# sozoluffy/TensorNetworks

Measured on AMD Instinct MI355X. Metric: ksd_gradient_steps_per_sec, higher is better.
Workload: dtype f64; 1 GPU; n16_L6_dense; n_qubits=16, layers=6, ansatz=hardware_efficient, params=288, gram=dense, bayesian_network=synthetic n=16 seed=0 (SURVEY 8d), optimizer=adam lr=0.005 cosine clip=10, parallelism=paramshift + gram row shard x1

## Files before the change

### tensornetworks_amd/csrc/plan.cpp

```cpp
#include "plan.hpp"

#include <algorithm>
#include <array>
#include <cstring>
#include <utility>

namespace bornvi {

int num_params(int ansatz, int n, int layers) {
  if (ansatz == 0 || ansatz == 1) return layers * 3 * n;
  if (ansatz == 2) return layers * 2 * n;
  return -1;
}

bool build_gate_list(int ansatz, int n, int layers, std::vector<Gate>& g) {
  g.clear();
  int p = 0;
  auto rot = [&](int kind, int w) { g.push_back({kind, w, -1, p++}); };
  if (ansatz == 0) {
    for (int i = 0; i < n; ++i) g.push_back({G_H, i, -1, -1});
    for (int l = 0; l < layers; ++l) {
      for (int i = 0; i < n; ++i) { rot(G_RX, i); rot(G_RY, i); rot(G_RZ, i); }
      if (n > 1) {
        for (int i = 0; i + 1 < n; ++i) g.push_back({G_CNOT, i, i + 1, -1});
// ... 180 lines not shown
}

std::vector<int> order_for_banks(std::vector<int> pos) {
  std::sort(pos.begin(), pos.end());
  std::vector<int> out;
  std::vector<char> used(pos.size(), 0);
  bool res_used[4] = {false, false, false, false};
  auto take = [&](auto pred) -> bool {
    for (size_t i = 0; i < pos.size(); ++i)
      if (!used[i] && pred(pos[i])) { used[i] = 1; out.push_back(pos[i]); res_used[pos[i] & 3] = true; return true; }
    return false;
  };
  for (int s = 0; s < 3 && out.size() < pos.size(); ++s)
    if (!take([&](int p) { return (p & 3) != 3 && !res_used[p & 3]; }))
      take([&](int) { return true; });
  if (out.size() < pos.size())
    if (!take([&](int p) { return (p & 3) == 3; })) take([&](int) { return true; });
  if (out.size() < pos.size() && out.size() >= 2) {
    int r0 = out[0] & 3, r1 = out[1] & 3;
    if (!take([&](int p) { return (p & 3) == r0 || (p & 3) == r1; })) take([&](int) { return true; });
  }
  for (size_t i = 0; i < pos.size(); ++i)
    if (!used[i]) out.push_back(pos[i]);
  return out;
}

void split_pass_ops(const std::vector<Op>& ops, const std::vector<int>& pass_ops, int n, bool is_init,
                    std::vector<int>& lead, std::vector<int>& core, std::vector<int>& trail) {
  lead.clear(); core.clear(); trail.clear();
  std::vector<char> touched(n, 0);
  std::vector<int> mid;
  for (int idx : pass_ops) {
    const Op& o = ops[idx];
    if (!is_init && o.kind == K_CX && !touched[o.a] && !touched[o.b]) { lead.push_back(idx); continue; }
    touched[o.a] = 1; if (o.b >= 0) touched[o.b] = 1;
    mid.push_back(idx);
  }
  std::fill(touched.begin(), touched.end(), 0);
  std::vector<int> trail_rev, core_rev;
  for (size_t q = mid.size(); q-- > 0;) {
    const Op& o = ops[mid[q]];
    if (o.kind == K_CX && !touched[o.a] && !touched[o.b]) { trail_rev.push_back(mid[q]); continue; }
    touched[o.a] = 1; if (o.b >= 0) touched[o.b] = 1;
    core_rev.push_back(mid[q]);
  }
  core.assign(core_rev.rbegin(), core_rev.rend());
  trail.assign(trail_rev.rbegin(), trail_rev.rend());
}

int count_stages(const std::vector<Op>& ops, const std::vector<int>& core, int n, int r, bool defer_cx3, bool read_map) {
  std::vector<int> pool = core, rest;
  int cnt = 0;
  while (!pool.empty()) {
    StageSel sel;
    stage_select(ops, pool, n, r, sel, rest, defer_cx3, read_map);
    if (sel.count() == 0) return 1 << 20;
    ++cnt;
    pool = rest;
  }
  return cnt;
}
bool pick_defer_policy(const std::vector<Op>& ops, const std::vector<int>& core, int n, int r, bool read_map) {
  return read_map && count_stages(ops, core, n, r, true, true) < count_stages(ops, core, n, r, false, true);
}

void first_last_stage_targets(const std::vector<Op>& ops, const std::vector<int>& pass_ops, int n, int r, bool is_init,
                              std::vector<int>& first_t, std::vector<int>& last_t, bool read_map) {
  std::vector<int> lead, core, trail, rest;
  split_pass_ops(ops, pass_ops, n, is_init, lead, core, trail);
  first_t.clear(); last_t.clear();
  std::vector<int> pool = core;
  bool first = true;
  const bool defer = pick_defer_policy(ops, core, n, r, read_map);
  while (!pool.empty()) {
    StageSel sel;
    stage_select(ops, pool, n, r, sel, rest, defer, read_map);
    if (sel.count() == 0) break;
    if (first) { first_t = sel.targets; first = false; }
    last_t = sel.targets;
    pool = rest;
  }
}

struct PassInfo {
  std::vector<int> ops;
  std::vector<int> targets;
  std::vector<int> local;
  std::vector<int> global;
  std::vector<int> lds_wire;
  std::vector<int> in_low;
  std::vector<int> out_low;
};

}

namespace {
struct BuildSpec {
  int n = 0;
  std::vector<Op> ops;
  std::vector<Fused> fused;
  int n_params = 0, n_gates = 0;
  bool in_state = false;
  bool out_state = false;
  std::vector<std::pair<int, int>> out_perm;
};
bool build_plan(const BuildSpec& spec, const PlanOptions& opt, Plan& plan, std::string& msg);
}

namespace {
bool make_plan_impl(int ansatz, int n, int layers, const PlanOptions& opt, Plan& plan, std::string& msg, std::vector<TailOp>* tail);
}

bool make_plan(int ansatz, int n, int layers, const PlanOptions& opt, Plan& plan, std::string& msg) {
  return make_plan_impl(ansatz, n, layers, opt, plan, msg, nullptr);
}

bool make_state_plan(int ansatz, int n, int layers, const PlanOptions& opt, Plan& plan, std::vector<TailOp>& tail, std::string& msg) {
  tail.clear();
  return make_plan_impl(ansatz, n, layers, opt, plan, msg, &tail);
}

namespace {
bool make_plan_impl(int ansatz, int n, int layers, const PlanOptions& opt, Plan& plan, std::string& msg, std::vector<TailOp>* tail) {
  if (n < 1 || n > MAX_PLAN_QUBITS) { msg = "num qubits must be in [1, " + std::to_string(MAX_PLAN_QUBITS) + "]"; return false; }
  if (layers < 0) { msg = "layers must be >= 0"; return false; }
  std::vector<Gate> gates;
  if (!build_gate_list(ansatz, n, layers, gates)) { msg = "unknown ansatz id"; return false; }
  BuildSpec spec;
  spec.n = n;
  fuse_gates(gates, n, spec.ops, spec.fused);
  {
    size_t last_u = spec.ops.size();
    while (last_u > 0 && spec.ops[last_u - 1].kind != K_U1) --last_u;
    for (size_t q = last_u; q < spec.ops.size(); ++q) {
      if (tail) tail->push_back({spec.ops[q].kind == K_CZ ? 1 : 0, spec.ops[q].a, spec.ops[q].b});
      else if (spec.ops[q].kind == K_CX) spec.out_perm.push_back({spec.ops[q].a, spec.ops[q].b});
    }
    spec.ops.resize(last_u);
  }
  spec.out_state = tail != nullptr;
  spec.n_params = num_params(ansatz, n, layers);
  spec.n_gates = (int)gates.size();
  if (opt.kmulti == 0 && n > opt.kmax && opt.kmax >= 13) {
    PlanOptions o11 = opt, o13 = opt;
    o11.kmulti = 11;
    o13.kmulti = 13;
    if (opt.r == 3) return build_plan(spec, o13, plan, msg);
    Plan p13;
    std::string m13;
    if (build_plan(spec, o13, p13, m13)) {
      FastTables ft;
      if ((build_fast_tables(p13, FAST_TABLE_MAX_BYTES, ft) && p13.fast_lds_bytes(ft.max_tab_rows) <= MAX_LDS_BYTES) ||
          n - o11.kmulti > 16) {
        plan = std::move(p13);
        return true;
      }
    }
    return build_plan(spec, o11, plan, msg);
  }
  return build_plan(spec, opt, plan, msg);
}
}

bool make_kron_plan(int n, const PlanOptions& opt, Plan& plan, std::string& msg) {
  if (n < 1 || n > MAX_PLAN_QUBITS) { msg = "num bits must be in [1, " + std::to_string(MAX_PLAN_QUBITS) + "]"; return false; }
  BuildSpec spec;
  spec.n = n;
  Fused f; f.fill(0xffffffffu); f[0] = 0; f[1] = 0;
  spec.fused.push_back(f);
  for (int w = n - 1; w >= 0; --w) spec.ops.push_back({K_U1, w, -1, 0});
  spec.in_state = spec.out_state = true;
  spec.n_gates = n;
  if (opt.kmulti == 0 && n - 12 > 16 && opt.kmax >= 13) {
    PlanOptions o13 = opt;
    o13.kmulti = 13;
    return build_plan(spec, o13, plan, msg);
  }
  return build_plan(spec, opt, plan, msg);
}

namespace {
bool build_plan(const BuildSpec& spec, const PlanOptions& opt, Plan& plan, std::string& msg) {
  const int n = spec.n;
  const std::vector<Op>& ops = spec.ops;
  const std::vector<Fused>& fused = spec.fused;
  const int kmulti = opt.kmulti > 0 ? opt.kmulti : (n <= 16 ? 11 : 12);
  const int k = (n <= opt.kmax) ? n : std::min(opt.kmax, kmulti);
  const int r = std::min(opt.r, k);
  if (r > 4) { msg = "at most 4 register wires"; return false; }
  int threads = 64;
  while (threads < (1 << (k - r))) threads <<= 1;
  if (threads > opt.max_threads) { msg = "tile needs more threads than allowed"; return false; }
  if (fused.size() > 65535) { msg = "too many fused gates"; return false; }

  std::vector<PassInfo> passes;
  {
    std::vector<int> pool(ops.size());
    for (size_t i = 0; i < ops.size(); ++i) pool[i] = (int)i;
    std::vector<int> sel, rest, tg;
    while (!pool.empty()) {
      choose_pass(ops, pool, n, k, sel, rest, tg);
      if (sel.empty()) { msg = "planner made no progress"; return false; }
      PassInfo pi; pi.ops = sel; pi.targets = tg;
      passes.push_back(pi);
      pool = rest;
    }
    if (passes.empty()) passes.push_back(PassInfo{});
  }
  const int lo_can = std::min(opt.lo, k);
  std::vector<int> canon_low;
  for (int p = 0; p < lo_can; ++p) canon_low.push_back(n - 1 - p);
  std::vector<int> canon_low_out = canon_low;
  {
    auto count_with = [&](int lo) {
      std::vector<char> in(n, 0);
      int cnt = 0;
      for (int w : passes.back().targets) { in[w] = 1; ++cnt; }
      for (int p = 0; p < lo; ++p) if (!in[n - 1 - p]) { in[n - 1 - p] = 1; ++cnt; }
      return cnt;
    };
    int lo_fit = -1;
    for (int lo = lo_can; lo >= std::min(3, lo_can); --lo)
      if (count_with(lo) <= k) { lo_fit = lo; break; }
    if (lo_fit < 0) passes.push_back(PassInfo{});
    else canon_low_out.resize(lo_fit);
  }
  if (spec.in_state) {
    std::vector<char> in(n, 0);
    int cnt = 0;
    for (int w : passes.front().targets) { in[w] = 1; ++cnt; }
    for (int w : canon_low) if (!in[w]) { in[w] = 1; ++cnt; }
    if (cnt > k) passes.insert(passes.begin(), PassInfo{});
  }
  const int np = (int)passes.size();
  for (int i = 0; i < np; ++i) {
    PassInfo& P = passes[i];
    std::vector<char> in(n, 0);
    auto add = [&](int w) { if (!in[w] && (int)P.local.size() < k) { in[w] = 1; P.local.push_back(w); } };
    for (int w : P.targets) add(w);
    if (i == np - 1) for (int w : canon_low_out) add(w);
    if (i == 0 && spec.in_state) for (int w : canon_low) add(w);
    if (i + 1 < np) for (int w : passes[i + 1].targets) add(w);
    if (i > 0) for (int w : passes[i - 1].local) add(w);
    for (int w = n - 1; w >= 0; --w) add(w);
    for (int w = 0; w < n; ++w) if (!in[w]) P.global.push_back(w);
  }
  if (spec.in_state) passes[0].in_low = canon_low;
  for (int i = 0; i < np; ++i) {
    PassInfo& P = passes[i];
    std::vector<char> placed(n, 0);
    for (int w : P.in_low) { P.lds_wire.push_back(w); placed[w] = 1; }
    std::vector<int> others;
    for (int w : P.local) if (!placed[w]) others.push_back(w);
    std::sort(others.begin(), others.end());
    for (int w : others) P.lds_wire.push_back(w);
    if (i == np - 1) { P.out_low = canon_low_out; break; }
    std::vector<char> nxt(n, 0);
    for (int w : passes[i + 1].local) nxt[w] = 1;
    std::vector<int> ldspos(n, -1);
    for (int j = 0; j < k; ++j) ldspos[P.lds_wire[j]] = j;
    std::vector<int> pos;
    for (int w : P.local) if (nxt[w]) pos.push_back(ldspos[w]);
    {
      std::vector<int> f_cur, l_cur, f_nxt, l_nxt;
      first_last_stage_targets(ops, P.ops, n, r, i == 0 && !spec.in_state, f_cur, l_cur, opt.use_read_map());
      first_last_stage_targets(ops, passes[i + 1].ops, n, r, false, f_nxt, l_nxt, opt.use_read_map());
      std::vector<char> busy(n, 0);
      for (int w : l_cur) busy[w] = 1;
      for (int w : f_nxt) busy[w] = 1;
      std::vector<int> quiet;
      for (int q : pos) if (!busy[P.lds_wire[q]]) quiet.push_back(q);
      if ((int)quiet.size() >= std::min(4, std::min(opt.lo, k))) pos = quiet;
    }
    pos = order_for_banks(pos);
    const int lo = std::min((int)pos.size(), std::min(opt.lo, k));
    for (int j = 0; j < lo; ++j) P.out_low.push_back(P.lds_wire[pos[j]]);
    passes[i + 1].in_low = P.out_low;
  }
  std::vector<std::vector<int>> layout(np, std::vector<int>(n, -1));
  for (int i = 0; i < np; ++i) {
    if (i == np - 1) { for (int w = 0; w < n; ++w) layout[i][w] = n - 1 - w; continue; }
    int p = 0;
    for (int w : passes[i].out_low) layout[i][w] = p++;
    if (opt.contig_out) {
      std::vector<char> nxt(n, 0);
      for (int w : passes[i + 1].local) nxt[w] = 1;
      for (int w : passes[i].local) if (layout[i][w] < 0 && nxt[w]) layout[i][w] = p++;
      for (int w : passes[i].local) if (layout[i][w] < 0) layout[i][w] = p++;
    }
    for (int w = 0; w < n; ++w) if (layout[i][w] < 0) layout[i][w] = p++;
  }
// ... 469 lines not shown
        const uint32_t* RWL = W.data() + rw_base + (size_t)(nst - 1) * per_stage;
        bool ok = (n + sh) <= 32;
        uint32_t basis[4] = {0, 0, 0, 0};
        for (int b = 0; b < r; ++b) basis[b] = phys_v(inv[W[hbase + FH_WORDS + (size_t)(nst - 1) * FS_WORDS + FS_WB + b] >> 4]) << sh;
        const uint32_t lanes_o = 1u << std::min<uint32_t>(P[PW_LO_OUT], 6u);
        const uint32_t runmask = (lanes_o << sh) - 1u;
        if (P[PW_LO_OUT] < 4u && !(pflags & PASS_FINAL)) ok = false;
        if ((pflags & PASS_FINAL) && P[PW_LO_OUT] < 3u) ok = false;
        for (uint32_t g = 0; g < ngl && ok; ++g) {
          uint32_t gslot = 0, gphys = 0;
          for (int m = 0; m < n - k; ++m) if (g >> m & 1) { gslot ^= thalf(PW_OUT_GMASK, m); gphys ^= P[PW_OUT_GCOL + m]; }
          for (uint32_t t = 0; t < (1u << kt2); ++t) {
            const uint32_t wslot = RWL[((size_t)g << kt2) + t] >> 16;
            W[tab + ((size_t)g << kt2) + t] = (phys_v(inv[wslot ^ gslot]) ^ gphys) << sh;
          }
          for (uint32_t t0 = 0; t0 < (1u << kt2) && ok; t0 += lanes_o) {
            uint32_t runs[2] = {0, 0};
            int nruns = 0;
            uint64_t seen = 0;
            for (uint32_t l = 0; l < lanes_o; ++l) {
              const uint32_t o = W[tab + ((size_t)g << kt2) + t0 + l];
              const uint32_t rb = o & ~runmask;
              int f = -1;
              for (int q = 0; q < nruns; ++q) if (runs[q] == rb) f = q;
              if (f < 0) { if (nruns == 2) { ok = false; break; } runs[nruns++] = rb; }
              seen |= 1ull << ((o >> sh) & (lanes_o - 1u));
            }
            if (nruns > ((pflags & PASS_FINAL) ? 2 : 1)) ok = false;
            if (seen != (lanes_o == 64 ? ~0ull : ((1ull << lanes_o) - 1ull))) ok = false;
          }
        }
        if (ok) {
          W[hbase + FH_OUT_TAB] = tab;
          for (int b = 0; b < r; ++b) W[hbase + FH_OUT_BASIS + b] = basis[b];
        } else {
          W.resize(tab);
        }
      }
    }
  }
  return true;
}


namespace {
inline uint32_t par32(uint32_t v) { return (uint32_t)__builtin_popcount(v) & 1u; }

struct StageEval {
  const uint32_t* S = nullptr;
  const uint32_t* tab = nullptr;
  const uint32_t* Qpre = nullptr;
  const uint32_t* Qpost = nullptr;
  uint32_t sri[3] = {0, 0, 0}, rpos[3] = {0, 0, 0};
  int k = 0, n = 0;
  uint32_t rw(uint32_t g, uint32_t t, uint32_t* e_out = nullptr, uint32_t* e2_out = nullptr) const {
    const uint32_t pb = tab[t] & 0xffffu, base = tab[t] >> 16;
    const uint32_t e = base | (g << k);
    uint32_t lflip = 0, sflip = 0, e2 = e;
    for (int b = 0; b < 3; ++b) {
      if (par32(e & S[8 + b])) lflip ^= sri[b];
      if (par32(e & S[12 + b])) { sflip ^= sri[b]; e2 |= 1u << rpos[b]; }
    }
    for (int p2 = 0; p2 < k; ++p2)
      if (S[48 + p2] && par32(e & S[48 + p2])) lflip ^= lds_swizzle(1u << p2);
    if (e_out) *e_out = e;
    if (e2_out) *e2_out = e2;
    return (pb ^ lflip) | ((pb ^ sflip) << 16);
  }
  uint32_t sign_bits(const uint32_t* Q, uint32_t e) const {
    uint32_t acc = 0;
    for (int q = 0; q < n; ++q) acc ^= ((e >> q) & 1u) & par32(e & Q[q]);
    uint32_t m = 0;
    for (int j = 0; j < 16; ++j) m |= (((Q[48] >> j) ^ acc ^ par32(e & Q[32 + j])) & 1u) << j;
    return m;
  }
  uint32_t sg(uint32_t g, uint32_t t) const {
    uint32_t e, e2;
    (void)rw(g, t, &e, &e2);
    return (Qpre ? sign_bits(Qpre, e) : 0u) | ((Qpost ? sign_bits(Qpost, e2) : 0u) << 16);
  }
};
}

bool build_compact_tables(const Plan& plan, CompactTables& out, std::string& msg) {
  out = CompactTables();
  const int n = plan.n, k = plan.k, r = plan.r;
  if (r != 3) { msg = "compact tables: the plan must have 3 register wires"; return false; }
  if (k < 6 || plan.threads != std::max(64, 1 << (k - 3)) || n - k > 16 || n > 27) { msg = "compact tables: tile below 2^6 or state too large"; return false; }
  const int kt = k - 3, gbits = n - k;
  const uint32_t T = 1u << kt, NW = std::max(T / 64u, 1u), ngl = 1u << gbits, ksize = 1u << k;
  std::vector<uint32_t>& W = out.words;
  auto fail = [&](const std::string& m) { msg = "compact tables: " + m; out = CompactTables(); return false; };
  for (int i = 0; i < plan.n_passes; ++i) {
    const uint32_t* P = plan.words.data() + plan.pass_off[i];
    const uint32_t nst = P[PW_NSTAGES];
    if (nst > (uint32_t)MAX_STAGES) return fail("too many stages");
    auto tbyte = [&](int table, int j) { return (P[table + (j >> 2)] >> (8 * (j & 3))) & 0xffu; };
    auto thalf = [&](int table, int j) { return (P[table + (j >> 1)] >> (16 * (j & 1))) & 0xffffu; };
    const uint32_t pflags = P[PW_FLAGS];
    const int out_shift = (pflags & PASS_FINAL) ? 3 : 4;
    std::vector<StageEval> SE(nst);
    uint32_t sign_pre = 0, sign_post = 0;
    {
      const uint32_t* S = P + PW_STAGES;
      for (uint32_t s = 0; s < nst; ++s) {
        const uint32_t hdr = S[0], sflags = (hdr >> 8) & 0xffu, rho = S[1];
        if ((hdr & 0xffu) != 3u) return fail("a stage with r != 3");
        StageEval& E = SE[s];
        E.S = S; E.k = k; E.n = n;
        for (int b = 0; b < 3; ++b) { E.rpos[b] = (rho >> (8 * b)) & 0xffu; E.sri[b] = lds_swizzle(1u << E.rpos[b]); }
        E.Qpre = (sflags & STAGE_SIGN_PRE) ? S + STAGE_HDR_WORDS : nullptr;
        E.Qpost = (sflags & STAGE_SIGN_POST) ? S + STAGE_HDR_WORDS + (E.Qpre ? SIGNQ_WORDS : 0) : nullptr;
        E.tab = S + STAGE_HDR_WORDS + (E.Qpre ? SIGNQ_WORDS : 0) + (E.Qpost ? SIGNQ_WORDS : 0);
        if (E.Qpre) sign_pre |= 1u << s;
        if (E.Qpost) sign_post |= 1u << s;
        S += hdr >> 16;
      }
    }
    const uint32_t sign_any = sign_pre | sign_post;
    const uint32_t nsign = (uint32_t)__builtin_popcount(sign_any);
    const uint32_t nrows = nst + nsign + CR_EXTRA;
    const uint32_t hb = (uint32_t)W.size();
    out.pass_off.push_back(hb);
    W.resize(hb + CH_WORDS + (size_t)nst * CS_WORDS, 0);
    W[hb + CH_NSTAGES] = nst; W[hb + CH_NROWS] = nrows; W[hb + CH_NSIGN] = nsign;
    W[hb + CH_SIGN_PRE] = sign_pre; W[hb + CH_SIGN_POST] = sign_post; W[hb + CH_NWAVES] = NW;
    for (uint32_t s = 0; s < nst; ++s) {
      const uint32_t* S = SE[s].S;
      const uint32_t sflags = (S[0] >> 8) & 0xffu;
      const uint32_t fi[4] = {S[6] & 0xffffu, S[6] >> 16, S[7] & 0xffffu, S[7] >> 16};
      uint32_t ngt = 0;
      while (ngt < 3 && fi[ngt] != 0xffffu) ++ngt;
      for (uint32_t b = ngt; b < 4; ++b) if (fi[b] != 0xffffu) return fail("gates not on register bits 0 .. ng-1");
      uint32_t* CS = W.data() + hb + CH_WORDS + (size_t)s * CS_WORDS;
      CS[CS_KIND] = ngt | ((sflags & STAGE_SIGN_PRE) ? 8u : 0u) | ((sflags & STAGE_SIGN_POST) ? 16u : 0u);
      CS[CS_CROSS] = (sflags & STAGE_CROSS_READ) ? 1u : 0u;
      for (int b = 0; b < 3; ++b) {
        CS[CS_RB + b] = S[16 + (1 << b)] << 4; CS[CS_WB + b] = S[32 + (1 << b)] << 4;
        CS[CS_MAT + b] = (fi[b] != 0xffffu ? fi[b] : 0u) * 64u;
      }
      for (int j = 0; j < 8; ++j) {
        uint32_t lr = 0, lw = 0;
        for (int b = 0; b < 3; ++b) if (j >> b & 1) { lr ^= S[16 + (1 << b)]; lw ^= S[32 + (1 << b)]; }
        if (lr != S[16 + j] || lw != S[32 + j]) return fail("slot offsets not linear in the slot number");
      }
    }
    W[hb + CH_MAT_OFF] = (uint32_t)W.size() - hb;
    {
      uint32_t nmat = 0;
      for (uint32_t s = 0; s < nst; ++s) {
        const uint32_t* S = SE[s].S;
        const uint32_t fi[3] = {S[6] & 0xffffu, S[6] >> 16, S[7] & 0xffffu};
        for (int b = 0; b < 3; ++b) if (fi[b] != 0xffffu) { W.push_back(fi[b] * 64u); ++nmat; }
      }
      W[hb + CH_NMAT] = nmat;
    }
    for (int m = 0; m < 3; ++m) {
      W[hb + CH_IN_STEP_N + m] = 16u << tbyte(PW_IN_PHYS, kt + m);
      W[hb + CH_FILL_STEP + m] = thalf(PW_IN_MASK, kt + m);
      W[hb + CH_DRAIN_STEP + m] = thalf(PW_OUT_MASK, kt + m);
      W[hb + CH_OUT_STEP_N + m] = P[PW_OUT_COL + kt + m] << out_shift;
    }
    std::vector<uint32_t> inv_in, inv_out;
    bool ok_in = false, ok_out = false;
    uint32_t in_basis[3] = {0, 0, 0}, out_basis[3] = {0, 0, 0};
    auto in_slot_lin = [&](uint32_t u) { uint32_t o = 0; for (int j = 0; j < k; ++j) if (u >> j & 1) o ^= thalf(PW_IN_MASK, j); return o; };
    auto in_phys_u = [&](uint32_t u) { uint32_t o = 0; for (int j = 0; j < k; ++j) if (u >> j & 1) o |= 1u << tbyte(PW_IN_PHYS, j); return o; };
    auto out_slot_lin = [&](uint32_t v) { uint32_t o = 0; for (int j = 0; j < k; ++j) if (v >> j & 1) o ^= thalf(PW_OUT_MASK, j); return o; };
    auto out_phys_v = [&](uint32_t v) { uint32_t o = 0; for (int j = 0; j < k; ++j) if (v >> j & 1) o ^= P[PW_OUT_COL + j]; return o; };
    auto g_in = [&](uint32_t g, uint32_t& gslot, uint32_t& gphys) {
      gslot = gphys = 0;
      for (int m = 0; m < gbits; ++m) if (g >> m & 1) { gslot ^= thalf(PW_IN_GMASK, m); gphys |= 1u << tbyte(PW_IN_GPHYS, m); }
    };
    auto g_out = [&](uint32_t g, uint32_t& gslot, uint32_t& gphys) {
      gslot = gphys = 0;
      for (int m = 0; m < gbits; ++m) if (g >> m & 1) { gslot ^= thalf(PW_OUT_GMASK, m); gphys ^= P[PW_OUT_GCOL + m]; }
// ... 7 lines not shown
      uint32_t gslot, gphys;
      g_out(g, gslot, gphys);
      return (out_phys_v(inv_out[(SE[nst - 1].rw(g, t) >> 16) ^ gslot]) ^ gphys) << out_shift;
    };
    if (nst > 0) {
      const uint32_t f0 = (SE[0].S[0] >> 8) & 0xffu, fl = (SE[nst - 1].S[0] >> 8) & 0xffu;
      if ((f0 & STAGE_FROM_HBM) && !(pflags & PASS_INIT)) {
        inv_in.assign(ksize, 0);
        for (uint32_t u = 0; u < ksize; ++u) inv_in[in_slot_lin(u)] = u;
        for (int b = 0; b < 3; ++b) in_basis[b] = in_phys_u(inv_in[W[hb + CH_WORDS + CS_RB + b] >> 4]) << 4;
        const uint32_t lanes = 1u << std::min<uint32_t>(P[PW_LO_IN], 6u);
        ok_in = P[PW_LO_IN] >= 4u && lanes <= T;
        const uint32_t runmask = lanes * 16u - 1u;
        std::vector<uint32_t> row(T);
        for (uint32_t g = 0; g < ngl && ok_in; ++g) {
          for (uint32_t t = 0; t < T; ++t) row[t] = in_d(g, t);
          for (uint32_t t0 = 0; t0 < T && ok_in; t0 += lanes) {
            const uint32_t base_run = row[t0] & ~runmask;
            uint64_t seen = 0;
            for (uint32_t l = 0; l < lanes; ++l) {
              if ((row[t0 + l] & ~runmask) != base_run) ok_in = false;
              seen |= 1ull << ((row[t0 + l] >> 4) & (lanes - 1u));
            }
            if (seen != (lanes == 64 ? ~0ull : ((1ull << lanes) - 1ull))) ok_in = false;
          }
        }
        for (int b = 0; b < 3; ++b) if (in_basis[b] & ((16u << std::min<uint32_t>(P[PW_LO_IN], 6u)) - 1u)) ok_in = false;
      }
      if (fl & STAGE_TO_HBM) {
        inv_out.assign(ksize, 0);
        for (uint32_t v = 0; v < ksize; ++v) inv_out[out_slot_lin(v)] = v;
        for (int b = 0; b < 3; ++b) out_basis[b] = out_phys_v(inv_out[W[hb + CH_WORDS + (size_t)(nst - 1) * CS_WORDS + CS_WB + b] >> 4]) << out_shift;
        ok_out = (n + out_shift) <= 32;
        const uint32_t lanes_o = 1u << std::min<uint32_t>(P[PW_LO_OUT], 6u);
        const uint32_t runmask = (lanes_o << out_shift) - 1u;
        if (P[PW_LO_OUT] < 4u && !(pflags & PASS_FINAL)) ok_out = false;
        if ((pflags & PASS_FINAL) && P[PW_LO_OUT] < 3u) ok_out = false;
        if (lanes_o > T) ok_out = false;
        std::vector<uint32_t> row(T);
        for (uint32_t g = 0; g < ngl && ok_out; ++g) {
          for (uint32_t t = 0; t < T; ++t) row[t] = out_d(g, t);
          for (uint32_t t0 = 0; t0 < T && ok_out; t0 += lanes_o) {
            uint32_t runs[2] = {0, 0};
            int nruns = 0;
            uint64_t seen = 0;
            for (uint32_t l = 0; l < lanes_o; ++l) {
              const uint32_t o = row[t0 + l], rb = o & ~runmask;
              int f = -1;
              for (int q = 0; q < nruns; ++q) if (runs[q] == rb) f = q;
              if (f < 0) { if (nruns == 2) { ok_out = false; break; } runs[nruns++] = rb; }
              seen |= 1ull << ((o >> out_shift) & (lanes_o - 1u));
            }
            if (nruns > ((pflags & PASS_FINAL) ? 2 : 1)) ok_out = false;
            if (seen != (lanes_o == 64 ? ~0ull : ((1ull << lanes_o) - 1ull))) ok_out = false;
          }
        }
      }
    }
    W[hb + CH_DIRECT] = (ok_in ? 1u : 0u) | (ok_out ? 2u : 0u);
    for (int b = 0; b < 3; ++b) { W[hb + CH_IN_STEP_D + b] = ok_in ? in_basis[b] : 0u; W[hb + CH_OUT_STEP_D + b] = ok_out ? out_basis[b] : 0u; }
    if (ok_in && i == 1 && (plan.words[plan.pass_off[0] + PW_FLAGS] & PASS_INIT) && plan.n_passes > 2) {
      const uint32_t* P0 = plan.words.data() + plan.pass_off[0];
      uint32_t zbits = 0;
      for (int m = 0; m < gbits; ++m) zbits |= 16u << ((P0[PW_OUT_GPHYS + (m >> 2)] >> (8 * (m & 3))) & 0xffu);
      uint32_t in_base = 0, in_slot = 0;
      for (uint32_t g = 0; g < ngl; ++g)
        for (uint32_t t = 0; t < T; ++t) in_base |= in_d(g, t) & zbits;
      for (int b = 0; b < 3; ++b) in_slot |= in_basis[b] & zbits;
      const uint32_t zs = in_slot & ~in_base;
      if (zs) {
        uint32_t zslots = 0;
        for (int j = 0; j < 8; ++j) {
          uint32_t off = 0;
          for (int b = 0; b < 3; ++b) if (j >> b & 1) off ^= in_basis[b];
          if (off & zs) zslots |= 1u << j;
        }
        uint32_t gmask0 = 0;
        for (int m = 0; m < gbits; ++m)
          if (zs & (16u << ((P0[PW_OUT_GPHYS + (m >> 2)] >> (8 * (m & 3))) & 0xffu))) gmask0 |= 1u << m;
        W[hb + CH_ZINFO] = zslots;
        W[out.pass_off[0] + CH_ZINFO] = gmask0;
      }
    }
    const uint32_t lo_in = P[PW_LO_IN];
    auto row_eval = [&](uint32_t row, uint32_t g, uint32_t t) -> uint32_t {
      if (row < nst) return SE[row].rw(g, t);
      if (row < nst + nsign) {
        uint32_t s = 0, seen = 0;
        for (;; ++s) if ((sign_any >> s) & 1u) { if (seen == row - nst) break; ++seen; }
        return SE[s].sg(g, t);
      }
      switch ((int)(row - nst - nsign)) {
        case CR_IN_D: return ok_in ? in_d(g, t) : 0u;
        case CR_OUT_D: return ok_out ? out_d(g, t) : 0u;
        case CR_IN_N: {
          uint32_t o = t & ((1u << lo_in) - 1u);
          for (int j = (int)lo_in; j < kt; ++j) o |= ((t >> j) & 1u) << tbyte(PW_IN_PHYS, j);
          for (int m = 0; m < gbits; ++m) o |= ((g >> m) & 1u) << tbyte(PW_IN_GPHYS, m);
          return o << 4;
        }
        case CR_OUT_N: {
          uint32_t o = 0;
          for (int j = 0; j < kt; ++j) if (t >> j & 1) o ^= P[PW_OUT_COL + j];
          for (int m = 0; m < gbits; ++m) if (g >> m & 1) o ^= P[PW_OUT_GCOL + m];
          return o << out_shift;
        }
        default: {
          uint32_t a = 0, b2 = 0;
          for (int j = 0; j < kt; ++j) if (t >> j & 1) { a ^= thalf(PW_IN_MASK, j); b2 ^= thalf(PW_OUT_MASK, j); }
          for (int m = 0; m < gbits; ++m) if (g >> m & 1) { a ^= thalf(PW_IN_GMASK, m); b2 ^= thalf(PW_OUT_GMASK, m); }
          return a | (b2 << 16);
        }
      }
    };
    const uint32_t lane_off = (uint32_t)W.size() - hb;
    W.resize(W.size() + (size_t)nrows * 64, 0);
    const uint32_t uni_off = (uint32_t)W.size() - hb;
    W.resize(W.size() + (size_t)ngl * nrows * NW, 0);
    const uint32_t mask_off = (uint32_t)W.size() - hb;
    W.resize(W.size() + (size_t)ngl * (nsign ? nsign : 1u) * NW, 0);
    W[hb + CH_LANE_OFF] = lane_off; W[hb + CH_UNI_OFF] = uni_off; W[hb + CH_MASK_OFF] = mask_off;
    for (uint32_t row = 0; row < nrows; ++row) {
      const bool is_sign = row >= nst && row < nst + nsign;
      const uint32_t f00 = row_eval(row, 0, 0);
      uint32_t* LANE = W.data() + hb + lane_off + (size_t)row * 64;
      for (uint32_t l = 0; l < 64; ++l) LANE[l] = l < T ? row_eval(row, 0, l) : 0u;
      for (uint32_t g = 0; g < ngl; ++g)
        for (uint32_t w = 0; w < NW; ++w) {
          const uint32_t fgw = row_eval(row, g, 64u * w);
          W[hb + uni_off + ((size_t)g * nrows + row) * NW + w] = fgw ^ f00;
          if (is_sign) {
            uint32_t mpre = 0, mpost = 0;
            for (int b = 0; b < 6 && b < kt; ++b) {
              const uint32_t d = row_eval(row, g, 64u * w + (1u << b)) ^ LANE[1u << b] ^ fgw ^ f00;
              mpre |= (d & 1u) << b;
              mpost |= ((d >> 16) & 1u) << b;
            }
            W[hb + mask_off + ((size_t)g * nsign + (row - nst)) * NW + w] = mpre | (mpost << 8);
          }
        }
      const uint32_t gstep = ((size_t)ngl * T <= ((size_t)1 << 22)) ? 1u : ngl / 64u;
      for (uint32_t g = 0; g < ngl; g += gstep)
        for (uint32_t t = 0; t < T; ++t) {
          const uint32_t l = t & 63u, w = t >> 6;
          uint32_t v = LANE[l] ^ W[hb + uni_off + ((size_t)g * nrows + row) * NW + w];
          if (is_sign) {
            const uint32_t mk = W[hb + mask_off + ((size_t)g * nsign + (row - nst)) * NW + w];
            if (par32(l & (mk & 0xffu))) v ^= 0x0000ffffu;
            if (par32(l & (mk >> 8))) v ^= 0xffff0000u;
          }
          if (v != row_eval(row, g, t)) return fail("a table word is not affine in (tile row, thread): pass " + std::to_string(i) + " row " + std::to_string(row));
        }
    }
    out.max_rows = std::max(out.max_rows, (int)nrows);
    out.max_sign = std::max(out.max_sign, (int)nsign);
    out.max_stages = std::max(out.max_stages, (int)nst);
  }
  if (W.size() >= (size_t)0x7fffffffu) return fail("tables too large");
  return true;
}

}
```

### tensornetworks_amd/csrc/plan.hpp

```cpp
#pragma once
#include <algorithm>
#include <cstddef>
#include <cstdint>
#include <string>
#include <vector>

namespace bornvi {

enum GateKind : int { G_H = 0, G_RX = 1, G_RY = 2, G_RZ = 3, G_CNOT = 4, G_CZ = 5 };

struct Gate {
  int kind;
  int w0;
  int w1;
  int param;
};

int num_params(int ansatz, int n, int layers);
bool build_gate_list(int ansatz, int n, int layers, std::vector<Gate>& out);

constexpr uint32_t PLAN_MAGIC = 0x424e5649u;
enum PlanHeader : int {
  PH_MAGIC = 0, PH_N, PH_K, PH_NPASSES, PH_NFUSED, PH_NPARAMS, PH_OFF_FUSED, PH_OFF_PASSTAB,
  PH_TOTAL, PH_THREADS, PH_R, PH_NGATES, PH_SIZE = 16
// ... 27 lines not shown
constexpr uint32_t STAGE_SIGN_PRE = 1u;
constexpr uint32_t STAGE_SIGN_POST = 2u;
constexpr uint32_t STAGE_FROM_HBM = 4u;
constexpr uint32_t STAGE_TO_HBM = 8u;
constexpr uint32_t STAGE_CROSS_READ = 16u;
constexpr int SIGNQ_WORDS = 49;

#if defined(__HIPCC__)
#define BORNVI_HD __host__ __device__
#else
#define BORNVI_HD
#endif
BORNVI_HD inline uint32_t lds_swizzle(uint32_t l) { return l ^ (((l >> 4) ^ (l >> 8) ^ (l >> 12)) & 15u); }

constexpr size_t FAST_TABLE_MAX_BYTES = (size_t)256 << 20;
constexpr size_t MAX_LDS_BYTES = 160 * 1024;

struct PlanOptions {
  int kmax = 13;
  int kmulti = 0;
  int r = 3;
  int lo = 6;
  int max_threads = 1024;
  int contig_out = 1;
  int read_map = -1;
  bool use_read_map() const { return read_map < 0 ? r == 3 : read_map != 0; }
};

struct Plan {
  int n = 0, k = 0, r = 0, n_passes = 0, n_fused = 0, n_params = 0, threads = 0, n_gates = 0;
  int max_stages = 0;
  std::vector<uint32_t> words;
  std::vector<uint32_t> pass_off;
  std::vector<int> param_first_pass;
  size_t lds_bytes() const { return (size_t(1) << k) * 16 + (((size_t)(max_stages > 0 ? max_stages : 1) * STAGE_MATS_BYTES + 511) / 512) * 512; }
  size_t fast_mats_bytes() const { return (size_t)(max_stages > 0 ? max_stages : 1) * STAGE_MATS_BYTES; }
  size_t fast_lds_tab_off() const { return (size_t(1) << k) * 16 + fast_mats_bytes(); }
  size_t fast_tab_bytes(int tab_rows) const { return ((size_t)(tab_rows + 4) * ((size_t)1 << (k - 4)) * 4 + 15) / 16 * 16; }
  size_t fast_lds_mats2_off(int tab_rows) const { return fast_lds_tab_off() + fast_tab_bytes(tab_rows); }
  size_t fast_lds_bytes(int tab_rows) const { return fast_lds_mats2_off(tab_rows) + fast_mats_bytes(); }
};

enum FastHeader : int { FH_NSTAGES = 0, FH_RW_BASE, FH_SG_BASE, FH_SIGN_PRE, FH_SIGN_POST, FH_IN_TAB, FH_OUT_TAB,
                        FH_ZINFO = 7,
                        FH_IN_BASIS = 8, FH_OUT_BASIS = 12, FH_WORDS = 16 };
enum FastStage : int { FS_FI01 = 0, FS_FI23, FS_RB = 2, FS_WB = 6, FS_KIND = 10, FS_CROSS = 11 , FS_WORDS = 16 };

constexpr bool fast_stage_kind_supported(uint32_t kind) { return (kind & 7u) <= 4u && (kind >> 5) == 0u; }

struct FastTables {
  int r = 4;
  std::vector<uint32_t> words;
  std::vector<uint32_t> pass_off;
  bool any_sign = false;
  int max_tab_rows = 1;
};
bool build_fast_tables(const Plan& plan, size_t max_bytes, FastTables& out);

enum CompactHeader : int {
  CH_NSTAGES = 0, CH_NROWS, CH_NSIGN, CH_SIGN_PRE, CH_SIGN_POST,
  CH_DIRECT,
  CH_ZINFO,
  CH_NWAVES, CH_MAT_OFF, CH_LANE_OFF, CH_UNI_OFF, CH_MASK_OFF,
  CH_NMAT = 30,
  CH_IN_STEP_D = 12,
  CH_IN_STEP_N = 15,
  CH_FILL_STEP = 18,
  CH_DRAIN_STEP = 21,
  CH_OUT_STEP_D = 24,
  CH_OUT_STEP_N = 27,
  CH_WORDS = 32
};
enum CompactStage : int { CS_KIND = 0, CS_CROSS, CS_RB = 2, CS_WB = 5, CS_MAT = 8, CS_WORDS = 12 };
enum CompactRow : int { CR_IN_D = 0, CR_IN_N, CR_OUT_D, CR_OUT_N, CR_SLOT, CR_EXTRA = 5 };
struct CompactTables {
  std::vector<uint32_t> words;
  std::vector<uint32_t> pass_off;
  int max_rows = 0, max_sign = 0, max_stages = 0;
  size_t lds_bytes(int k) const {
    const size_t nw = std::max<size_t>(((size_t)1 << (k - 3)) / 64, 1);
    return ((size_t)16 << k) + (size_t)max_rows * 64 * 4 + (size_t)max_rows * nw * 4 + (size_t)(max_sign > 0 ? max_sign : 1) * nw * 4 + 8 + nw * 8 + 64;
  }
};
bool build_compact_tables(const Plan& plan, CompactTables& out, std::string& msg);

constexpr int MAX_PLAN_QUBITS = 29;
bool make_plan(int ansatz, int n, int layers, const PlanOptions& opt, Plan& out, std::string& msg);
struct TailOp { int is_cz, a, b; };
bool make_state_plan(int ansatz, int n, int layers, const PlanOptions& opt, Plan& out, std::vector<TailOp>& tail, std::string& msg);
bool make_kron_plan(int n, const PlanOptions& opt, Plan& out, std::string& msg);

}
```

Baseline: 233.5 steps/s.

## Add beam search over pass partitions to reduce plan passes and stages

```diff
diff --git a/tensornetworks_amd/csrc/plan.cpp b/tensornetworks_amd/csrc/plan.cpp
--- a/tensornetworks_amd/csrc/plan.cpp
+++ b/tensornetworks_amd/csrc/plan.cpp
@@ -286,6 +286,218 @@
   }
 }
 
+struct PassPick { std::vector<int> ops, targets; };
+
+int pass_stage_count(const std::vector<Op>& ops, const std::vector<int>& pass_ops, int n, int r, bool is_init, bool read_map) {
+  std::vector<int> lead, core, trail;
+  split_pass_ops(ops, pass_ops, n, is_init, lead, core, trail);
+  int c = count_stages(ops, core, n, r, false, read_map);
+  if (read_map) c = std::min(c, count_stages(ops, core, n, r, true, true));
+  return c;
+}
+
+bool last_pass_fits(const std::vector<int>& targets, int n, int k, int lo_can) {
+  for (int lo = lo_can; lo >= std::min(3, lo_can); --lo) {
+    uint32_t in = 0;
+    for (int w : targets) in |= 1u << w;
+    for (int p = 0; p < lo; ++p) in |= 1u << (n - 1 - p);
+    if (__builtin_popcount(in) <= k) return true;
+  }
+  return false;
+}
+
+void mask_select(const std::vector<Op>& ops, const std::vector<int>& pool, uint32_t allowed, uint32_t all_wires,
+                 std::vector<int>& sel, int& bound_sel) {
+  uint32_t blocked = 0;
+  sel.clear(); bound_sel = 0;
+  for (int idx : pool) {
+    const Op& o = ops[idx];
+    const uint32_t wires = (1u << o.a) | (o.b >= 0 ? 1u << o.b : 0u);
+    const int t = op_target(o);
+    if ((blocked & wires) || (t >= 0 && !((allowed >> t) & 1u))) {
+      blocked |= wires;
+      if (blocked == all_wires) break;
+    } else {
+      if (t >= 0) ++bound_sel;
+      sel.push_back(idx);
+    }
+  }
+}
+
+struct VecIndex {
+  std::unordered_map<uint64_t, std::vector<int>> buckets;
+  std::vector<std::vector<int>> keys;
+  static uint64_t hash(const std::vector<int>& v, uint64_t salt) {
+    uint64_t h = 1469598103934665603ull ^ salt;
+    for (int x : v) h = (h ^ (uint64_t)(uint32_t)x) * 1099511628211ull;
+    return h;
+  }
+  int find_or_add(const std::vector<int>& v, uint64_t salt, bool& added) {
+    std::vector<int>& b = buckets[hash(v, salt)];
+    for (int id : b) if (keys[(size_t)id] == v) { added = false; return id; }
+    keys.push_back(v);
+    b.push_back((int)keys.size() - 1);
+    added = true;
+    return (int)keys.size() - 1;
+  }
+  void clear() { buckets.clear(); keys.clear(); }
+};
+
+constexpr int MAX_SUBSETS = 1024;
+void candidate_sets(int n, int k, std::vector<uint32_t>& out) {
+  out.clear();
+  std::vector<uint32_t> windows;
+  for (int s0 = 0; s0 < n; ++s0) {
+    uint32_t a = 0;
+    for (int j = 0; j < k; ++j) a |= 1u << ((s0 + j) % n);
+    windows.push_back(a);
+  }
+  out = windows;
+  double nsub = 1;
+  for (int j = 1; j <= n - k; ++j) nsub = nsub * (double)(n - (n - k) + j) / (double)j;
+  if (nsub <= (double)MAX_SUBSETS) {
+    for (uint32_t a = 0; a < (1u << n); ++a)
+      if (__builtin_popcount(a) == k) out.push_back(a);
+  } else {
+    for (uint32_t w : windows)
+      for (int i = 0; i < n; ++i)
+        if ((w >> i) & 1u)
+          for (int j = 0; j < n; ++j)
+            if (!((w >> j) & 1u)) out.push_back((w & ~(1u << i)) | (1u << j));
+  }
+  std::vector<uint32_t> uniq;
+  std::vector<uint32_t> seen;
+  for (uint32_t a : out) {
+    auto it = std::lower_bound(seen.begin(), seen.end(), a);
+    if (it != seen.end() && *it == a) continue;
+    seen.insert(it, a);
+    uniq.push_back(a);
+  }
+  out.swap(uniq);
+}
+
+struct SearchNode {
+  std::vector<int> pool;
+  int parent = -1;
+  int stages = 0;
+  int bound_left = 0;
+  PassPick pick;
+};
+
+bool search_passes(const std::vector<Op>& ops, int n, int k, int r, int lo_can, bool init0, bool read_map,
+                   const std::vector<PassPick>& prefix, int max_passes, std::vector<PassPick>& out, int& out_passes, int& out_stages) {
+  std::vector<uint32_t> cands;
+  candidate_sets(n, k, cands);
+  const double node_work = (double)(cands.size() + 1) * (double)std::max<size_t>(ops.size(), 1) * (double)std::max(max_passes, 1);
+  const int beam = (int)std::max(4.0, std::min(64.0, 1.5e8 / node_work));
+  std::vector<std::vector<SearchNode>> levels(1);
+  {
+    SearchNode root;
+    std::vector<char> done(ops.size(), 0);
+    for (size_t d = 0; d < prefix.size(); ++d) {
+      for (int idx : prefix[d].ops) done[(size_t)idx] = 1;
+      root.stages += pass_stage_count(ops, prefix[d].ops, n, r, d == 0 && init0, read_map);
+    }
+    for (size_t i = 0; i < ops.size(); ++i)
+      if (!done[i]) { root.pool.push_back((int)i); if (op_target(ops[i]) >= 0) ++root.bound_left; }
+    if (root.pool.empty()) return false;
+    levels[0].push_back(std::move(root));
+  }
+  VecIndex stage_keys;
+  std::vector<int> stage_vals;
+  int best_passes = max_passes + 1, best_stages = 0, best_level = -1, best_node = -1;
+  PassPick best_last;
+  std::vector<int> sel, rest, gs, gr, gt;
+  VecIndex seen_here, next_keys;
+  const uint32_t all_wires = n >= 32 ? 0xffffffffu : (1u << n) - 1u;
+  for (int depth = (int)prefix.size(); depth < max_passes; ++depth) {
+    const std::vector<SearchNode>& cur = levels.back();
+    std::vector<SearchNode> next;
+    next_keys.clear();
+    const bool is_init = depth == 0 && init0;
+    for (size_t ni = 0; ni < cur.size(); ++ni) {
+      const SearchNode& N = cur[ni];
+      seen_here.clear();
+      greedy_select(ops, N.pool, n, k, gs, gr, gt);
+      uint32_t gmask = 0;
+      for (int w : gt) gmask |= 1u << w;
+      for (int w = n - 1, cnt = (int)gt.size(); w >= 0 && cnt < k; --w) if (!((gmask >> w) & 1u)) { gmask |= 1u << w; ++cnt; }
+      for (size_t ci = 0; ci <= cands.size(); ++ci) {
+        const uint32_t allowed = ci == 0 ? gmask : cands[ci - 1];
+        int bound_sel;
+        mask_select(ops, N.pool, allowed, all_wires, sel, bound_sel);
+        if (sel.empty()) continue;
+        bool added;
+        seen_here.find_or_add(sel, 0, added);
+        if (!added) continue;
+        rest.clear();
+        for (size_t a = 0, b = 0; a < N.pool.size(); ++a) {
+          if (b < sel.size() && sel[b] == N.pool[a]) ++b;
+          else rest.push_back(N.pool[a]);
+        }
+        const int bound_left = N.bound_left - bound_sel;
+        const int sid = stage_keys.find_or_add(sel, is_init ? 1 : 0, added);
+        if (added) stage_vals.push_back(pass_stage_count(ops, sel, n, r, is_init, read_map));
+        const int stages = N.stages + stage_vals[(size_t)sid];
+        std::vector<int> targets;
+        for (int idx : sel) {
+          const int t = op_target(ops[idx]);
+          if (t >= 0 && std::find(targets.begin(), targets.end(), t) == targets.end()) targets.push_back(t);
+        }
+        if (rest.empty()) {
+          const int passes = depth + 1 + (last_pass_fits(targets, n, k, lo_can) ? 0 : 1);
+          if (passes < best_passes || (passes == best_passes && stages < best_stages)) {
+            best_passes = passes; best_stages = stages; best_level = (int)levels.size() - 1; best_node = (int)ni;
+            best_last.ops = sel; best_last.targets = targets;
+          }
+          continue;
+        }
+        if (depth + 1 >= max_passes) continue;
+        const int id = next_keys.find_or_add(rest, 0, added);
+        if (added) {
+          SearchNode C;
+          C.pool = rest; C.parent = (int)ni; C.stages = stages; C.bound_left = bound_left;
+          C.pick.ops = sel; C.pick.targets = targets;
+          next.push_back(std::move(C));
+        } else if (stages < next[(size_t)id].stages) {
+          SearchNode& C = next[(size_t)id];
+          C.parent = (int)ni; C.stages = stages; C.pick.ops = sel; C.pick.targets = targets;
+        }
+      }
+    }
+    if (is_init) { stage_keys.clear(); stage_vals.clear(); }
+    if (next.empty()) break;
+    if ((int)next.size() > beam) {
+      std::vector<int> by_left(next.size()), by_cost(next.size());
+      for (size_t i = 0; i < next.size(); ++i) by_left[i] = by_cost[i] = (int)i;
+      std::stable_sort(by_left.begin(), by_left.end(), [&](int a, int b) {
+        return next[(size_t)a].bound_left != next[(size_t)b].bound_left ? next[(size_t)a].bound_left < next[(size_t)b].bound_left
+                                                                        : next[(size_t)a].stages < next[(size_t)b].stages; });
+      std::stable_sort(by_cost.begin(), by_cost.end(), [&](int a, int b) {
+        return 3 * next[(size_t)a].stages + next[(size_t)a].bound_left < 3 * next[(size_t)b].stages + next[(size_t)b].bound_left; });
+      std::vector<char> keep(next.size(), 0);
+      int kept = 0;
+      for (size_t i = 0; i < next.size() && kept < beam / 2; ++i) if (!keep[(size_t)by_left[i]]) { keep[(size_t)by_left[i]] = 1; ++kept; }
+      for (size_t i = 0; i < next.size() && kept < beam; ++i) if (!keep[(size_t)by_cost[i]]) { keep[(size_t)by_cost[i]] = 1; ++kept; }
+      std::vector<SearchNode> pruned;
+      for (size_t i = 0; i < next.size(); ++i) if (keep[i]) pruned.push_back(std::move(next[i]));
+      next.swap(pruned);
+    }
+    levels.push_back(std::move(next));
+  }
+  if (best_level < 0) return false;
+  std::vector<PassPick> rev;
+  rev.push_back(best_last);
+  for (int lv = best_level, id = best_node; lv > 0; --lv) {
+    rev.push_back(levels[(size_t)lv][(size_t)id].pick);
+    id = levels[(size_t)lv][(size_t)id].parent;
+  }
+  out = prefix;
+  out.insert(out.end(), rev.rbegin(), rev.rend());
+  out_passes = best_passes; out_stages = best_stages;
+  return true;
+}
+
 struct PassInfo {
   std::vector<int> ops;
   std::vector<int> targets;
@@ -309,6 +521,8 @@
   std::vector<std::pair<int, int>> out_perm;
 };
 bool build_plan(const BuildSpec& spec, const PlanOptions& opt, Plan& plan, std::string& msg);
+bool assemble_plan(const BuildSpec& spec, const PlanOptions& opt, int k, int r, int threads, const std::vector<PassPick>& picks,
+                   Plan& plan, std::string& msg);
 }
 
 namespace {
@@ -397,7 +611,7 @@
   if (threads > opt.max_threads) { msg = "tile needs more threads than allowed"; return false; }
   if (fused.size() > 65535) { msg = "too many fused gates"; return false; }
 
-  std::vector<PassInfo> passes;
+  std::vector<PassPick> heur;
   {
     std::vector<int> pool(ops.size());
     for (size_t i = 0; i < ops.size(); ++i) pool[i] = (int)i;
@@ -405,12 +619,51 @@
     while (!pool.empty()) {
       choose_pass(ops, pool, n, k, sel, rest, tg);
       if (sel.empty()) { msg = "planner made no progress"; return false; }
-      PassInfo pi; pi.ops = sel; pi.targets = tg;
-      passes.push_back(pi);
+      heur.push_back(PassPick{sel, tg});
       pool = rest;
     }
-    if (passes.empty()) passes.push_back(PassInfo{});
-  }
+  }
+  if (!assemble_plan(spec, opt, k, r, threads, heur, plan, msg)) return false;
+  if (r != 3 || k >= n || spec.in_state || heur.size() < 2) return true;
+  auto plan_cost = [&](const Plan& p, long& cost) {
+    CompactTables ct;
+    std::string m;
+    if (!build_compact_tables(p, ct, m, true)) return false;
+    long stages = 0;
+    for (int i = 0; i < p.n_passes; ++i) stages += (long)p.words[p.pass_off[(size_t)i] + PW_NSTAGES];
+    const int skipped_bits = __builtin_popcount(ct.words[ct.pass_off[0] + CH_ZINFO]);
+    const int zero_slots = p.n_passes > 1 ? __builtin_popcount(ct.words[ct.pass_off[1] + CH_ZINFO]) : 0;
+    const long written = 1024 >> std::min(skipped_bits, 10), loaded = 128 * (8 - zero_slots);
+    cost = 22 * 1024 * stages + 775 * (written + loaded) / 10;
+    return true;
+  };
+  long best_cost = 0;
+  if (!plan_cost(plan, best_cost)) return true;
+  const int lo_can0 = std::min(opt.lo, k);
+  for (size_t keep = 0; keep <= 1 && keep + 1 < heur.size(); ++keep) {
+    std::vector<PassPick> prefix(heur.begin(), heur.begin() + (long)keep), found;
+    int fp = 0, fs = 0;
+    if (!search_passes(ops, n, k, r, lo_can0, !spec.in_state, opt.use_read_map(), prefix, plan.n_passes, found, fp, fs)) continue;
+    Plan cand;
+    std::string m;
+    long cost = 0;
+    if (!assemble_plan(spec, opt, k, r, threads, found, cand, m) || !plan_cost(cand, cost)) continue;
+    if (cand.n_passes < plan.n_passes || (cand.n_passes == plan.n_passes && cost < best_cost)) {
+      plan = std::move(cand);
+      best_cost = cost;
+    }
+  }
+  return true;
+}
+
+bool assemble_plan(const BuildSpec& spec, const PlanOptions& opt, int k, int r, int threads, const std::vector<PassPick>& picks,
+                   Plan& plan, std::string& msg) {
+  const int n = spec.n;
+  const std::vector<Op>& ops = spec.ops;
+  const std::vector<Fused>& fused = spec.fused;
+  std::vector<PassInfo> passes;
+  for (const PassPick& pk : picks) { PassInfo pi; pi.ops = pk.ops; pi.targets = pk.targets; passes.push_back(pi); }
+  if (passes.empty()) passes.push_back(PassInfo{});
   const int lo_can = std::min(opt.lo, k);
   std::vector<int> canon_low;
   for (int p = 0; p < lo_can; ++p) canon_low.push_back(n - 1 - p);
@@ -1046,8 +1299,9 @@
 };
 }
 
-bool build_compact_tables(const Plan& plan, CompactTables& out, std::string& msg) {
+bool build_compact_tables(const Plan& plan, CompactTables& out, std::string& msg, bool zero_support_only) {
   out = CompactTables();
+  const int n_tab_passes = zero_support_only ? std::min(2, plan.n_passes) : plan.n_passes;
   const int n = plan.n, k = plan.k, r = plan.r;
   if (r != 3) { msg = "compact tables: the plan must have 3 register wires"; return false; }
   if (k < 6 || plan.threads != std::max(64, 1 << (k - 3)) || n - k > 16 || n > 27) { msg = "compact tables: tile below 2^6 or state too large"; return false; }
@@ -1055,7 +1309,7 @@
   const uint32_t T = 1u << kt, NW = std::max(T / 64u, 1u), ngl = 1u << gbits, ksize = 1u << k;
   std::vector<uint32_t>& W = out.words;
   auto fail = [&](const std::string& m) { msg = "compact tables: " + m; out = CompactTables(); return false; };
-  for (int i = 0; i < plan.n_passes; ++i) {
+  for (int i = 0; i < n_tab_passes; ++i) {
     const uint32_t* P = plan.words.data() + plan.pass_off[i];
     const uint32_t nst = P[PW_NSTAGES];
     if (nst > (uint32_t)MAX_STAGES) return fail("too many stages");
@@ -1229,6 +1483,7 @@
         W[out.pass_off[0] + CH_ZINFO] = gmask0;
       }
     }
+    if (zero_support_only) continue;
     const uint32_t lo_in = P[PW_LO_IN];
     auto row_eval = [&](uint32_t row, uint32_t g, uint32_t t) -> uint32_t {
       if (row < nst) return SE[row].rw(g, t);
diff --git a/tensornetworks_amd/csrc/plan.hpp b/tensornetworks_amd/csrc/plan.hpp
--- a/tensornetworks_amd/csrc/plan.hpp
+++ b/tensornetworks_amd/csrc/plan.hpp
@@ -133,7 +133,7 @@
     return ((size_t)16 << k) + (size_t)max_rows * 64 * 4 + (size_t)max_rows * nw * 4 + (size_t)(max_sign > 0 ? max_sign : 1) * nw * 4 + 8 + nw * 8 + 64;
   }
 };
-bool build_compact_tables(const Plan& plan, CompactTables& out, std::string& msg);
+bool build_compact_tables(const Plan& plan, CompactTables& out, std::string& msg, bool zero_support_only = false);
 
 constexpr int MAX_PLAN_QUBITS = 29;
 bool make_plan(int ansatz, int n, int layers, const PlanOptions& opt, Plan& out, std::string& msg);
```

Result: no change. 233.2 steps/s (-0.1%).
